# DerryHub/BEVFormer_tensorrt

Measured on AMD Instinct MI355X. Metric: frames/sec BEVFormer-base bs=1 fp16 end-to-end on MI355X (re-hosted model, random weights, synthetic 6-camera frames), higher is better.
Workload: dtype f16

## Files before the change

### bevformer_tensorrt_amd/csrc/capi.hip

```cpp
#include <string.h>

#include "common.h"

extern "C" const char *bevops_version(void) { return "bevops-hip 0.1 (gfx950)"; }

extern "C" const char *bevops_status_string(int status) {
  switch (status) {
    case BEVOPS_SUCCESS: return "success";
    case BEVOPS_FAILURE: return "failure (kernel launch error)";
    case BEVOPS_BAD_PARAM: return "bad parameter";
    case BEVOPS_NOT_SUPPORTED: return "dtype/shape combination not supported";
    case BEVOPS_NOT_INITIALIZED: return "not initialized";
    default: return "unknown status";
  }
}

namespace {
struct Entry {
  const char *name;
  void *fn;
};
const Entry kTable[] = {
    {"bevops_msda_forward", (void *)&bevops_msda_forward},
    {"bevops_msda_forward_ws", (void *)&bevops_msda_forward_ws},
// ... 55 lines not shown
    {"bevops_upsample_bilinear_concat_nhwc", (void *)&bevops_upsample_bilinear_concat_nhwc},
    {"bevops_tsa_split", (void *)&bevops_tsa_split},
    {"bevops_queue_mean2", (void *)&bevops_queue_mean2},
    {"bevops_tsgemm_f16", (void *)&bevops_tsgemm_f16},
    {"bevops_tsgemm_s8", (void *)&bevops_tsgemm_s8},
    {"bevops_tsgemm_s8_ln", (void *)&bevops_tsgemm_s8_ln},
    {"bevops_tsgemm_tile_rows", (void *)&bevops_tsgemm_tile_rows},
    {"bevops_tsgemm_f16_ln", (void *)&bevops_tsgemm_f16_ln},
    {"bevops_tsgemm_f16_grouped", (void *)&bevops_tsgemm_f16_grouped},
    {"bevops_mha_selfattn_f16", (void *)&bevops_mha_selfattn_f16},
    {"bevops_mha_selfattn_max_queries", (void *)&bevops_mha_selfattn_max_queries},
    {"bevops_value_proj_packed_size", (void *)&bevops_value_proj_packed_size},
    {"bevops_value_proj_packed", (void *)&bevops_value_proj_packed},
    {"bevops_value_pack_planes", (void *)&bevops_value_pack_planes},
    {"bevops_sca_prepacked_workspace_size", (void *)&bevops_sca_prepacked_workspace_size},
    {"bevops_sca_forward_prepacked", (void *)&bevops_sca_forward_prepacked},
    {"bevops_sca_plan_size", (void *)&bevops_sca_plan_size},
    {"bevops_sca_plan_build", (void *)&bevops_sca_plan_build},
    {"bevops_sca_forward_planned", (void *)&bevops_sca_forward_planned},
    {"bevops_point_sampling", (void *)&bevops_point_sampling},
    {"bevops_feat_embed_nhwc", (void *)&bevops_feat_embed_nhwc},
    {"bevops_linear_bias_act", (void *)&bevops_linear_bias_act},
    {"bevops_linear_tune", (void *)&bevops_linear_tune},
    {"bevops_quantize_rows", (void *)&bevops_quantize_rows},
    {"bevops_dequantize_rows", (void *)&bevops_dequantize_rows},
    {"bevops_linear_int8", (void *)&bevops_linear_int8},
    {"bevops_linear_int8_fused", (void *)&bevops_linear_int8_fused},
    {"bevops_tile_gemm_f16", (void *)&bevops_tile_gemm_f16},
    {"bevops_tile_gemm_f16_dst", (void *)&bevops_tile_gemm_f16_dst},
    {"bevops_small_gemm_f16_dst", (void *)&bevops_small_gemm_f16_dst},
    {"bevops_small_gemm_f16", (void *)&bevops_small_gemm_f16},
    {"bevops_conv_tile_f16", (void *)&bevops_conv_tile_f16},
    {"bevops_conv3x3_c64_f16", (void *)&bevops_conv3x3_c64_f16},
    {"bevops_refine_reference_points", (void *)&bevops_refine_reference_points},
    {"bevops_decode_boxes", (void *)&bevops_decode_boxes},
    {"bevops_conv_tile_int8_fused", (void *)&bevops_conv_tile_int8_fused},
    {"bevops_linear_int8_chain", (void *)&bevops_linear_int8_chain},
    {"bevops_conv_tile_int8", (void *)&bevops_conv_tile_int8},
    {"bevops_bias_relu_maxpool_nhwc_int8", (void *)&bevops_bias_relu_maxpool_nhwc_int8},
    {"bevops_mdconv_int8_nhwc_workspace_size", (void *)&bevops_mdconv_int8_nhwc_workspace_size},
    {"bevops_mdconv_forward_int8_nhwc", (void *)&bevops_mdconv_forward_int8_nhwc},
    {"bevops_image_normalize_pad", (void *)&bevops_image_normalize_pad},
    {"bevops_image_normalize_resize_pad", (void *)&bevops_image_normalize_resize_pad},
    {"bevops_image_resize_plan_size", (void *)&bevops_image_resize_plan_size},
    {"bevops_image_resize_plan_build", (void *)&bevops_image_resize_plan_build},
    {"bevops_image_resize_crop_normalize", (void *)&bevops_image_resize_crop_normalize},
    {"bevops_msda_packed_size", (void *)&bevops_msda_packed_size},
    {"bevops_msda_pack_value", (void *)&bevops_msda_pack_value},
    {"bevops_msda_forward_prepacked", (void *)&bevops_msda_forward_prepacked},
    {"bevops_linear_workspace_size", (void *)&bevops_linear_workspace_size},
    {"bevops_msda_workspace_size_shapes", (void *)&bevops_msda_workspace_size_shapes},
    {"bevops_sca_workspace_size", (void *)&bevops_sca_workspace_size},
    {"bevops_mdconv_forward_packed", (void *)&bevops_mdconv_forward_packed},
    {"bevops_mdconv_pack_weight", (void *)&bevops_mdconv_pack_weight},
    {"bevops_mdconv_packed_weight_size", (void *)&bevops_mdconv_packed_weight_size},
    {"bevops_conv3x3_c32_pack_weight", (void *)&bevops_conv3x3_c32_pack_weight},
    {"bevops_conv3x3_c32_packed_weight_size", (void *)&bevops_conv3x3_c32_packed_weight_size},
    {"bevops_layer_norm", (void *)&bevops_layer_norm},
    {"bevops_calib_state_size", (void *)&bevops_calib_state_size},
    {"bevops_calib_collect", (void *)&bevops_calib_collect},
    {"bevops_calib_threshold_workspace_size", (void *)&bevops_calib_threshold_workspace_size},
    {"bevops_calib_threshold", (void *)&bevops_calib_threshold},
};
}

extern "C" void *bevops_query(const char *name) {
// ... 6 lines not shown
```

### bevformer_tensorrt_amd/functions/__init__.py

```python
from .multi_scale_deformable_attn import (
    multi_scale_deformable_attn,
    multi_scale_deformable_attn2,
    multi_scale_deformable_attn_int8,
    multi_scale_deformable_attn_local,
    msda_pack_value,
    multi_scale_deformable_attn_prepacked,
)
from .rotate import rotate, rotate2, rotate_int8, rotate_hwc
from .grid_sampler import grid_sampler, grid_sampler2, grid_sampler_int8
from .bev_pool_v2 import bev_pool_v2, bev_pool_v2_2, bev_pool_v2_int8
from .modulated_deformable_conv2d import (modulated_deformable_conv2d, modulated_deformable_conv2d2,
                                          modulated_deformable_conv2d_int8, modulated_deformable_conv2d_nhwc,
                                          bias_act_nhwc_, bias_relu_maxpool_nhwc, conv_offset_nhwc, upsample_add_nhwc_,
                                          feat_embed_nhwc)
from .spatial_cross_attention import (spatial_cross_attention_sample, spatial_cross_attention_projected,
                                      spatial_cross_attention_plan)
from .linear import (linear_bias_act, layer_norm, quantize_rows, dequantize_rows, linear_int8, tsgemm, tsgemm_ln, tsgemm_grouped, tile_gemm, tile_gemm_dst, small_gemm, small_gemm_dst,
                     dense_auto, tsa_split, queue_mean2)
from .int8_chain import linear_int8_chain, linear_int8_ln
from .conv import conv_nhwc, conv3x3_nhwc, conv3x3_auto, conv3x3_c64, conv_int8_nhwc, stem_conv_pool
from .image import (image_normalize_pad, padded_size, bevdet_test_augmentation, bevdet_post_transform, image_resize_plan,
                    image_resize_crop_normalize, BEVFORMER_IMAGE_PIPELINES, scaled_size, scale_lidar2img,
                    image_normalize_resize_pad)
from .point_sampling import point_sampling
from .attention import self_attention_qkv
from .refine import refine_reference_points, decode_boxes
from .multi_head_attn import qkv, qkv2
from .inverse import inverse
from .decode import nms_free_decode, centerpoint_decode
from .nms import bev_nms, nms_bev, circle_nms, bev_iou
from .decode2d import centernet_decode, yolox_decode, box_nms
from .lss_prepare import lss_voxel_prepare, lss_lidar_coor, bev_pool_v2_indirect
from .calibrate import calib_state_size, calib_collect, calib_threshold
from .bev_half import lss_depth_split, upsample_bilinear_concat_nhwc
from ..utils.register import TRT_FUNCTIONS

TRT_FUNCTIONS.register_module(module=multi_scale_deformable_attn)
TRT_FUNCTIONS.register_module(module=multi_scale_deformable_attn2)
TRT_FUNCTIONS.register_module(module=multi_scale_deformable_attn_int8)
for _f in (rotate, rotate2, rotate_int8, grid_sampler, grid_sampler2, grid_sampler_int8,
           bev_pool_v2, bev_pool_v2_2, bev_pool_v2_int8, modulated_deformable_conv2d,
           modulated_deformable_conv2d2, modulated_deformable_conv2d_int8,
           spatial_cross_attention_sample, inverse, qkv, qkv2):
    TRT_FUNCTIONS.register_module(module=_f)

__all__ = [
    "multi_scale_deformable_attn",
    "multi_scale_deformable_attn2",
    "multi_scale_deformable_attn_int8",
    "rotate", "rotate2", "rotate_int8",
    "grid_sampler", "grid_sampler2", "grid_sampler_int8",
    "bev_pool_v2", "bev_pool_v2_2", "bev_pool_v2_int8",
    "modulated_deformable_conv2d", "modulated_deformable_conv2d2", "modulated_deformable_conv2d_int8",
    "inverse", "qkv", "qkv2",
    "nms_free_decode", "centerpoint_decode",
    "bev_nms", "nms_bev", "circle_nms", "bev_iou",
    "centernet_decode", "yolox_decode", "box_nms",
    "lss_voxel_prepare", "lss_lidar_coor", "bev_pool_v2_indirect",
    "calib_state_size", "calib_collect", "calib_threshold",
    "bevdet_test_augmentation", "bevdet_post_transform", "image_resize_plan", "image_resize_crop_normalize",
    "BEVFORMER_IMAGE_PIPELINES", "scaled_size", "scale_lidar2img", "image_normalize_resize_pad",
    "spatial_cross_attention_sample", "spatial_cross_attention_projected", "spatial_cross_attention_plan", "modulated_deformable_conv2d_nhwc", "bias_act_nhwc_", "linear_bias_act", "layer_norm", "rotate_hwc", "conv_offset_nhwc", "upsample_add_nhwc_", "feat_embed_nhwc",
    "msda_pack_value", "multi_scale_deformable_attn_prepacked", "multi_scale_deformable_attn_local", "image_normalize_pad", "padded_size", "quantize_rows", "dequantize_rows", "linear_int8", "tsgemm", "tsgemm_ln", "tsgemm_grouped", "tile_gemm", "tile_gemm_dst", "small_gemm_dst", "small_gemm", "dense_auto", "tsa_split", "queue_mean2", "conv_nhwc", "conv3x3_nhwc", "conv3x3_auto", "conv3x3_c64", "conv_int8_nhwc", "bias_relu_maxpool_nhwc", "stem_conv_pool", "point_sampling", "self_attention_qkv", "refine_reference_points", "decode_boxes",
    "linear_int8_chain", "linear_int8_ln",
    "lss_depth_split", "upsample_bilinear_concat_nhwc",
]
```

### bevformer_tensorrt_amd/functions/conv.py

```python
import os

import torch
import torch.nn.functional as F

from ..utils import lib as _lib
from .modulated_deformable_conv2d import bias_act_nhwc_
from .multi_scale_deformable_attn import _TensorCache

_PACKED = _TensorCache()
_CHOICE = {}
CONV_LOG = []
CONV_MISSES = []
HALO = {"enabled": os.environ.get("BEVOPS_CONV_HALO", "1") == "1"}


def pack_taps(weight):
    hit = _PACKED.get(weight)
    if hit is None:
        hit = _PACKED.put(weight, weight.detach().permute(0, 2, 3, 1).contiguous())
    return hit


def conv_nhwc(x, weight, bias=None, relu=False, residual=None, stride=1):
    assert x.is_cuda and x.dtype == torch.float16 and x.dim() == 4 and weight.shape[2] == weight.shape[3]
    assert x.is_contiguous(memory_format=torch.channels_last)
    B, Cin, H, W = x.shape
    Cout, k = weight.shape[0], weight.shape[2]
    if weight.shape[1] != Cin:
        raise ValueError("weight does not match the input channels")
    wt = pack_taps(weight)
    Ho, Wo = (H + 2 * (k // 2) - k) // stride + 1, (W + 2 * (k // 2) - k) // stride + 1
    out = torch.empty((B, Cout, Ho, Wo), dtype=x.dtype, device=x.device, memory_format=torch.channels_last)
    if residual is not None:
        assert residual.shape == out.shape and residual.dtype == x.dtype
        assert residual.is_contiguous(memory_format=torch.channels_last)
    if bias is not None:
        bias = bias.to(torch.float16).contiguous()
    if B == 0:
        return out
    handle = _lib.load_library()
    with torch.cuda.device(x.device):
        st = handle.bevops_conv_tile_f16(x.data_ptr(), wt.data_ptr(), bias.data_ptr() if bias is not None else None,
                                         residual.data_ptr() if residual is not None else None, out.data_ptr(),
                                         B, H, W, Cin, Cout, k, int(stride), int(bool(relu)),
                                         _lib.current_stream_ptr(x.device))
    _lib.check(st, "bevops_conv_tile_f16")
    return out


def conv3x3_c64(x, weight, bias=None, relu=False, residual=None, stride=1):
    assert x.is_cuda and x.dtype == torch.float16 and x.dim() == 4
    assert x.is_contiguous(memory_format=torch.channels_last)
    B, Cin, H, W = x.shape
    Cout = weight.shape[0]
    if residual is not None or stride != 1 or tuple(weight.shape[1:]) != (Cin, 3, 3):
        raise _lib.BevopsError("bevops_conv3x3_c64_f16: 3x3 / stride 1 layers without identity rows only", _lib.NOT_SUPPORTED)
    wt = pack_taps(weight)
    out = torch.empty((B, Cout, H, W), dtype=x.dtype, device=x.device, memory_format=torch.channels_last)
    if bias is not None:
        bias = bias.to(torch.float16).contiguous()
    if B == 0:
        return out
    handle = _lib.load_library()
    with torch.cuda.device(x.device):
        st = handle.bevops_conv3x3_c64_f16(x.data_ptr(), wt.data_ptr(), bias.data_ptr() if bias is not None else None,
                                           out.data_ptr(), B, H, W, Cin, Cout, int(bool(relu)),
                                           _lib.current_stream_ptr(x.device))
    _lib.check(st, "bevops_conv3x3_c64_f16")
    return out


def conv_int8_nhwc(x, scale_a, w_q_taps, scale_w, bias=None, relu=False, residual=None, stride=1):
    assert x.is_cuda and x.dtype == torch.float16 and x.dim() == 4 and w_q_taps.dtype == torch.int8
    assert x.is_contiguous(memory_format=torch.channels_last) and w_q_taps.is_contiguous()
    B, Cin, H, W = x.shape
    Cout, k = w_q_taps.shape[0], w_q_taps.shape[1]
    assert w_q_taps.shape == (Cout, k, k, Cin)
    Ho, Wo = (H + 2 * (k // 2) - k) // stride + 1, (W + 2 * (k // 2) - k) // stride + 1
    out = torch.empty((B, Cout, Ho, Wo), dtype=x.dtype, device=x.device, memory_format=torch.channels_last)
    if residual is not None:
        assert residual.shape == out.shape and residual.dtype == x.dtype
        assert residual.is_contiguous(memory_format=torch.channels_last)
    per_channel = torch.is_tensor(scale_w)
    ws = scale_w.float().contiguous() if per_channel else None
    b = bias.float().contiguous() if bias is not None else None
    if B == 0:
        return out
    handle = _lib.load_library()
    with torch.cuda.device(x.device):
        st = handle.bevops_conv_tile_int8_fused(
            x.data_ptr(), float(scale_a), w_q_taps.data_ptr(), ws.data_ptr() if per_channel else None,
            1.0 if per_channel else float(scale_w), b.data_ptr() if b is not None else None,
            residual.data_ptr() if residual is not None else None, out.data_ptr(), B, H, W, Cin, Cout, k, int(stride),
            int(bool(relu)), _lib.current_stream_ptr(x.device))
    _lib.check(st, "bevops_conv_tile_int8_fused")
    return out


def conv3x3_nhwc(x, weight, bias=None, relu=False, residual=None, stride=1):
    assert weight.shape[2:] == (3, 3)
    return conv_nhwc(x, weight, bias, relu, residual, stride)


def _library(x, weight, bias, relu, residual, stride=1):
    y = F.conv2d(x, weight, None, stride, weight.shape[2] // 2)
    if not y.is_contiguous(memory_format=torch.channels_last):
        y = y.contiguous(memory_format=torch.channels_last)
    return bias_act_nhwc_(y, bias, residual, relu)


def conv3x3_auto(x, weight, bias=None, relu=False, residual=None, stride=1):
    B, Cin, H, W = x.shape
    if B == 0 and Cin % 32 == 0:
        return conv_nhwc(x, weight, bias, relu, residual, stride)
    key = (str(x.device), B, H, W, Cin, weight.shape[0], weight.shape[2], stride, bool(relu), residual is not None)
    from .linear import DETERMINISTIC, _problem, _table
    halo_ok = HALO["enabled"] and Cin == 64 and weight.shape[0] == 64 and stride == 1 and residual is None \
        and weight.shape[2] == 3
    name = ("halo" if halo_ok else "tile") if (DETERMINISTIC["enabled"] and Cin % 32 == 0) else _CHOICE.get(key)
    if name is None:
        name = _table()["conv"].get(_problem(key))
        if name == "tile" and halo_ok:
            name = "halo"
        if name in ("tile", "library", "halo") and (name == "library" or Cin % 32 == 0) and (name != "halo" or halo_ok):
            _CHOICE[key] = name
        else:
            name = None
            if _problem(key) not in CONV_MISSES:
                CONV_MISSES.append(_problem(key))
    if name is None:
        if Cin % 32 != 0:
            name = _CHOICE[key] = "library"
        elif torch.cuda.is_current_stream_capturing() or os.environ.get("BEVOPS_DENSE_TUNE", "1") == "0":
            name = "library"
        else:
            from .linear import graph_time_us
            times = {}
            for cand, fn in (("tile", conv_nhwc), ("library", _library)) + ((("halo", conv3x3_c64),) if halo_ok else ()):
                for _ in range(2):
                    fn(x, weight, bias, relu, residual, stride)
                torch.cuda.synchronize()
                times[cand] = round(graph_time_us(lambda: fn(x, weight, bias, relu, residual, stride), 4, 3), 1)
            CONV_LOG.append((key, times))
            name = _CHOICE[key] = min(times, key=times.get)
    return {"tile": conv_nhwc, "halo": conv3x3_c64, "library": _library}[name](x, weight, bias, relu, residual, stride)


_STEM_PACKED = _TensorCache()
STEM_FUSED = {"enabled": os.environ.get("BEVOPS_STEM_FUSED", "1") != "0"}


def stem_conv_pool(x, weight, bias=None, scale_out=None):
    assert x.is_cuda and x.dtype == torch.float16 and x.dim() == 4 and x.is_contiguous()
    n, c, h, w = x.shape
    if tuple(weight.shape) != (64, 3, 7, 7) or c != 3 or w % 2:
        raise ValueError("stem_conv_pool: a 7x7 convolution from 3 to 64 channels on images of even width")
    handle = _lib.load_library()
    bstamp = None if bias is None else _TensorCache._stamp(bias)
    hit = _STEM_PACKED.get(weight)
    if hit is None or hit[0] != bstamp:
        wt = weight.detach().to(torch.float16).contiguous()
        bs = None if bias is None else bias.detach().to(torch.float16).contiguous()
        packed = torch.empty(handle.bevops_stem_packed_size(), dtype=torch.uint8, device=x.device)
        with torch.cuda.device(x.device):
            st = handle.bevops_stem_pack(_lib.F16, wt.data_ptr(), bs.data_ptr() if bs is not None else None,
                                         packed.data_ptr(), _lib.current_stream_ptr(x.device))
        _lib.check(st, "bevops_stem_pack")
        hit = _STEM_PACKED.put(weight, (bstamp, packed))
    hc, wc = (h - 1) // 2 + 1, (w - 1) // 2 + 1
    hp, wp = (hc - 1) // 2 + 1, (wc - 1) // 2 + 1
    out = torch.empty((n, 64, hp, wp), dtype=torch.float16 if scale_out is None else torch.int8, device=x.device,
                      memory_format=torch.channels_last)
    if n == 0:
        return out
    with torch.cuda.device(x.device):
        st = handle.bevops_stem_conv_pool(_lib.F16, _lib.F16 if scale_out is None else _lib.I8, x.data_ptr(),
                                          hit[1].data_ptr(), out.data_ptr(), n, h, w,
                                          0.0 if scale_out is None else float(scale_out),
# ... 5 lines not shown
```

### bevformer_tensorrt_amd/functions/linear.py

```python
import ctypes

import torch

from ..utils import lib as _lib
from ..utils import workspace as _ws

def _workspace(device, nbytes, stream):
    return _ws.lend("linear", nbytes, device, stream)


_TUNED = set()


def _tune_once(handle, key, args, x2, out_shape):
    import os
    _TUNED.add(key)
    if os.environ.get("BEVOPS_LINEAR_TUNE", "1") == "0":
        return
    scratch = torch.empty(out_shape, dtype=x2.dtype, device=x2.device)
    a = list(args)
    a[5] = scratch.data_ptr()
    handle.bevops_linear_tune(*a)


# ... 262 lines not shown
class _PerThreadFlag:

    def __init__(self):
        import threading
        self._tls = threading.local()

    def __getitem__(self, key):
        assert key == "enabled"
        return getattr(self._tls, "enabled", False)

    def __setitem__(self, key, value):
        assert key == "enabled"
        self._tls.enabled = bool(value)


DETERMINISTIC = _PerThreadFlag()
OWN_KERNELS = _PerThreadFlag()


_TABLE = {"loaded": False, "dense": {}, "conv": {}, "measured_dense": {}}


def _table():
    import json
    import os
    if not _TABLE["loaded"]:
        _TABLE["loaded"] = True
        path = os.path.join(os.path.dirname(os.path.dirname(os.path.abspath(__file__))), "dispatch_gfx950.json")
        if os.path.exists(path) and os.environ.get("BEVOPS_DENSE_TUNE", "") not in ("0", "1"):
            try:
                t = json.load(open(path))
                _TABLE["dense"], _TABLE["conv"] = t.get("dense", {}), t.get("conv", {})
                _TABLE["measured_dense"] = t.get("measured_us", {}).get("dense", {})
            except (OSError, ValueError):
                pass
    return _TABLE


def _problem(key):
    return ",".join(str(int(v)) if isinstance(v, bool) else str(v) for v in key[1:])


def _small_pays(M, N, K):
    return K % 64 == 0 and K <= 1024 and M * N <= 1024 * 512


def _dense_deterministic(N, K, M=1 << 30):
    if _small_pays(M, N, K):
        return "small"
    return "tsgemm" if (N % 256 == 0 and K % 64 == 0 and K >= 256) else "tile"


def _dense_own(key, N, K, M):
    times = _table().get("measured_dense", {}).get(_problem(key), {})
    own = {k: v for k, v in times.items() if k in ("tile", "tsgemm", "small") and k in _DENSE}
    return min(own, key=own.get) if own else _dense_deterministic(N, K, M)


def own_kernel_choice(device, M, N, K, relu, has_bias, has_res):
    return _dense_own((str(device), M, N, K, bool(relu), bool(has_bias), bool(has_res)), N, K, M)


def _dense_default(N, K, has_res):
    if N == 256 and K % 64 == 0 and K >= 256:
        return "tsgemm"
    return "blaslt"
# ... 104 lines not shown
```

### bevformer_tensorrt_amd/utils/lib.py

```python
import ctypes
import os

_PKG = os.path.dirname(os.path.dirname(os.path.abspath(__file__)))
_LIB = None

c_int, c_float, c_void_p, c_size_t = ctypes.c_int, ctypes.c_float, ctypes.c_void_p, ctypes.c_size_t

SIGNATURES = {
    "bevops_version": (ctypes.c_char_p, []),
    "bevops_status_string": (ctypes.c_char_p, [c_int]),
    "bevops_query": (c_void_p, [ctypes.c_char_p]),
    "bevops_msda_set_variant": (c_int, [c_int]),
    "bevops_msda_forward": (c_int, [c_int, c_void_p, c_void_p, c_void_p, c_void_p, c_int,
                                    c_void_p, c_void_p, c_void_p] + [c_int] * 8 +
                            [c_float] * 4 + [c_void_p]),
    "bevops_msda_workspace_size": (c_size_t, [c_int] * 8),
    "bevops_msda_workspace_size_shapes": (c_size_t, [c_int, c_void_p] + [c_int] * 7),
    "bevops_msda_forward_ws": (c_int, [c_int, c_void_p, c_void_p, c_void_p, c_void_p, c_int,
                                       c_void_p, c_void_p, c_void_p] + [c_int] * 8 +
                               [c_float] * 4 + [c_int, c_void_p, c_size_t, c_void_p]),
    "bevops_msda_packed_size": (c_size_t, [c_int, c_void_p] + [c_int] * 7),
    "bevops_msda_pack_value": (c_int, [c_int, c_int, c_void_p, c_void_p, c_void_p, c_size_t] + [c_int] * 7 + [c_void_p]),
    "bevops_msda_forward_prepacked": (c_int, [c_int, c_void_p, c_size_t, c_void_p, c_void_p, c_int, c_void_p, c_void_p,
                                              c_void_p] + [c_int] * 8 + [c_float] * 4 + [c_int, c_void_p]),
# ... 57 lines not shown
    "bevops_conv3x3_c32_packed_weight_size": (c_size_t, [c_int, c_int]),
    "bevops_conv3x3_c32_pack_weight": (c_int, [c_int, c_void_p, c_void_p, c_int, c_int, c_void_p]),
    "bevops_conv3x3_c32_forward_nhwc": (c_int, [c_int, c_void_p, c_void_p, c_void_p, c_void_p, c_int, c_int, c_int,
                                                c_int, c_void_p]),
    "bevops_rotate_set_variant": (c_int, [c_int]),
    "bevops_rotate_forward_hwc": (c_int, [c_int, c_void_p, c_void_p, c_void_p, c_int, c_void_p,
                                          c_int, c_int, c_int, c_int, c_void_p]),
    "bevops_layer_norm": (c_int, [c_int, c_void_p, c_void_p, c_void_p, c_void_p, c_size_t, c_int, c_float, c_void_p]),
    "bevops_linear_workspace_size": (c_size_t, []),
    "bevops_linear_bias_act": (c_int, [c_int] + [c_void_p] * 5 + [ctypes.c_longlong, c_int, c_int, c_int,
                                                                  c_void_p, c_size_t, c_void_p]),
    "bevops_image_normalize_pad": (c_int, [c_int, c_void_p, c_int, c_void_p] + [c_int] * 5 +
                                   [ctypes.POINTER(ctypes.c_double), ctypes.POINTER(ctypes.c_double), c_int, c_int, c_void_p]),
    "bevops_image_normalize_resize_pad": (c_int, [c_int, c_void_p, c_int, c_void_p] + [c_int] * 7 +
                                          [ctypes.POINTER(ctypes.c_double), ctypes.POINTER(ctypes.c_double), c_int, c_int,
                                           c_void_p]),
    "bevops_image_resize_plan_size": (c_size_t, [c_int] * 8),
    "bevops_image_resize_plan_build": (c_int, [c_int] * 8 + [c_void_p, c_size_t]),
    "bevops_image_resize_crop_normalize": (c_int, [c_void_p, c_void_p, c_size_t, c_int, c_void_p, c_void_p] + [c_int] * 10 +
                                           [ctypes.POINTER(ctypes.c_double), ctypes.POINTER(ctypes.c_double), c_int, c_int,
                                            c_int, c_void_p]),
    "bevops_quantize_rows": (c_int, [c_int, c_void_p, c_void_p, c_size_t, c_float, c_void_p]),
    "bevops_dequantize_rows": (c_int, [c_int, c_void_p, c_void_p, c_size_t, c_float, c_void_p]),
    "bevops_linear_int8": (c_int, [c_void_p, c_float, c_void_p, c_void_p, c_float, c_void_p, c_void_p, c_int, c_void_p,
                                   c_float, ctypes.c_longlong, c_int, c_int, c_int, c_void_p]),
    "bevops_linear_int8_fused": (c_int, [c_void_p, c_float, c_void_p, c_void_p, c_float, c_void_p, c_void_p, c_int, c_void_p,
                                         c_float, ctypes.c_longlong, c_int, c_int, c_int, c_void_p]),
    "bevops_small_gemm_f16": (c_int, [c_void_p] * 5 + [ctypes.c_longlong, c_int, c_int, c_int, c_void_p]),
    "bevops_tile_gemm_f16": (c_int, [c_void_p] * 5 + [ctypes.c_longlong, c_int, c_int, c_int, c_void_p]),
    "bevops_tile_gemm_f16_dst": (c_int, [c_void_p] * 4 + [c_int, ctypes.c_longlong, c_int, c_int, c_int, c_void_p]),
    "bevops_small_gemm_f16_dst": (c_int, [c_void_p] * 4 + [c_int, ctypes.c_longlong, c_int, c_int, c_int, c_void_p]),
    "bevops_conv_tile_f16": (c_int, [c_void_p] * 5 + [c_int] * 8 + [c_void_p]),
    "bevops_conv3x3_c64_f16": (c_int, [c_void_p] * 4 + [c_int] * 6 + [c_void_p]),
    "bevops_refine_reference_points": (c_int, [c_int] + [c_void_p] * 4 + [c_int] * 2 + [c_void_p] * 3),
    "bevops_decode_boxes": (c_int, [c_int] + [c_void_p] * 3 + [c_int] + [c_float] * 6 + [c_void_p] * 3),
    "bevops_bias_relu_maxpool_nhwc": (c_int, [c_int, c_void_p, c_void_p, c_void_p, c_int, c_int, c_int, c_int, c_void_p]),
    "bevops_stem_packed_size": (c_size_t, []),
    "bevops_stem_pack": (c_int, [c_int, c_void_p, c_void_p, c_void_p, c_void_p]),
    "bevops_stem_conv_pool": (c_int, [c_int, c_int, c_void_p, c_void_p, c_void_p, c_int, c_int, c_int, c_float, c_void_p]),
    "bevops_stem_set_variant": (c_int, [c_int]),
    "bevops_conv_tile_int8_fused": (c_int, [c_void_p, c_float, c_void_p, c_void_p, c_float, c_void_p, c_void_p, c_void_p]
                                    + [c_int] * 8 + [c_void_p]),
    "bevops_linear_int8_chain": (c_int, [c_void_p, c_int, c_float, c_void_p, c_void_p, c_float, c_void_p, c_void_p, c_int,
                                         c_float, c_int, c_void_p, c_float, ctypes.c_longlong, c_int, c_int, c_int, c_void_p]),
    "bevops_conv_tile_int8": (c_int, [c_void_p, c_float, c_void_p, c_void_p, c_float, c_void_p, c_void_p, c_int, c_void_p,
                                      c_float] + [c_int] * 8 + [c_void_p]),
    "bevops_bias_relu_maxpool_nhwc_int8": (c_int, [c_int, c_void_p, c_void_p, c_void_p, c_float, c_int, c_int, c_int, c_int,
                                                   c_void_p]),
    "bevops_mdconv_int8_nhwc_workspace_size": (c_size_t, []),
    "bevops_mdconv_forward_int8_nhwc": (c_int, [c_void_p, c_float, c_void_p, c_int, c_float, c_float, c_void_p, c_float,
                                                c_void_p, c_void_p, c_float, c_int, c_int, c_void_p, c_size_t] + [c_int] * 15 +
                                        [c_void_p]),
    "bevops_linear_tune": (c_int, [c_int] + [c_void_p] * 5 + [ctypes.c_longlong, c_int, c_int, c_int,
                                                              c_void_p, c_size_t, c_void_p]),
    "bevops_mdconv_packed_weight_size": (c_size_t, [c_int] * 5),
    "bevops_mdconv_pack_weight": (c_int, [c_int, c_void_p, c_void_p] + [c_int] * 4 + [c_void_p]),
    "bevops_grid_sampler_3d_forward": (c_int, [c_int, c_void_p, c_void_p, c_void_p] + [c_int] * 11 +
                                       [c_void_p]),
    "bevops_qkv_workspace_size": (c_size_t, [c_int] * 5),
    "bevops_qkv_forward": (c_int, [c_int, c_void_p, c_void_p, c_void_p, c_void_p] + [c_int] * 4 + [c_float] * 4 +
                           [c_void_p, c_size_t, c_void_p]),
    "bevops_inverse_forward": (c_int, [c_int, c_void_p, c_void_p, c_int, c_int, c_void_p]),
    "bevops_nms_free_decode": (c_int, [c_int] + [c_void_p] * 6 + [c_int] * 4 + [c_void_p, c_float, c_int, c_void_p]),
    "bevops_centerpoint_decode_workspace_size": (c_size_t, [c_int] * 5),
    "bevops_centerpoint_decode": (c_int, [c_int] + [c_void_p] * 11 + [c_int] * 5 + [c_float] * 5 +
                                  [c_void_p, c_float, c_int, c_int, c_void_p, c_size_t, c_void_p]),
# ... 75 lines not shown
```

### include/bevops.h

```cpp
#ifndef BEVOPS_H_
#define BEVOPS_H_

#include <stddef.h>
#include <stdint.h>

#ifdef __cplusplus
extern "C" {
#endif

typedef enum {
  BEVOPS_SUCCESS = 0,
  BEVOPS_FAILURE = 1,
  BEVOPS_BAD_PARAM = 2,
  BEVOPS_NOT_SUPPORTED = 3,
  BEVOPS_NOT_INITIALIZED = 4
} bevops_status_t;

typedef enum { BEVOPS_F32 = 0, BEVOPS_F16 = 1, BEVOPS_I8 = 2, BEVOPS_U8 = 3  } bevops_dtype_t;

typedef enum { BEVOPS_BILINEAR = 0, BEVOPS_NEAREST = 1, BEVOPS_BICUBIC = 2 } bevops_interp_t;
typedef enum { BEVOPS_PAD_ZEROS = 0, BEVOPS_PAD_BORDER = 1, BEVOPS_PAD_REFLECTION = 2 } bevops_pad_t;

const char *bevops_version(void);
const char *bevops_status_string(int status);
// ... 129 lines not shown
                     void *stream);
int bevops_queue_mean2(int dtype, const void *x, void *out, size_t count, void *stream);
int bevops_rotate_forward_hwc(int dtype, const void *img, const void *angle, const void *center,
                              int angle_dtype, void *output, int channels, int height, int width,
                              int interpolation, void *stream);
int bevops_layer_norm(int dtype, const void *x, const void *gamma, const void *beta, void *out,
                      size_t rows, int channels, float eps, void *stream);
int bevops_quantize_rows(int dtype, const void *x, void *q, size_t count, float scale, void *stream);
int bevops_dequantize_rows(int dtype, const void *q, void *out, size_t count, float scale, void *stream);
int bevops_linear_int8(const void *a_q, float scale_a, const void *w_q, const float *w_scales,
                       float scale_w, const float *bias, const void *residual, int out_dtype,
                       void *out, float scale_out, long long M, int N, int K, int relu, void *stream);
int bevops_linear_int8_fused(const void *x_f16, float scale_a, const void *w_q, const float *w_scales,
                             float scale_w, const float *bias, const void *residual, int out_dtype,
                             void *out, float scale_out, long long M, int N, int K, int relu, void *stream);
int bevops_tile_gemm_f16(const void *x, const void *weight, const void *bias, const void *residual,
                         void *out, long long M, int N, int K, int relu, void *stream);
typedef struct bevops_gemm_dst {
  int col_begin, col_end;
  void *out;
  long long out_pitch;
  const void *res;
  long long res_pitch;
} bevops_gemm_dst;
int bevops_tile_gemm_f16_dst(const void *x, const void *weight, const void *bias, const bevops_gemm_dst *dst, int num_dst,
                             long long M, int N, int K, int relu, void *stream);
int bevops_small_gemm_f16_dst(const void *x, const void *weight, const void *bias, const bevops_gemm_dst *dst, int num_dst,
                              long long M, int N, int K, int relu, void *stream);
int bevops_conv_tile_f16(const void *x, const void *weight_taps, const void *bias, const void *residual,
                         void *out, int B, int H, int W, int Cin, int Cout, int ksize, int stride, int relu,
                         void *stream);
int bevops_conv3x3_c64_f16(const void *x, const void *weight_taps, const void *bias, void *out, int B, int H, int W,
                           int Cin, int Cout, int relu, void *stream);
int bevops_refine_reference_points(int dtype, const void *tmp, const void *reference_points, void *new_reference_points,
                                   void *reference_xy, int num_query, int tmp_stride, const void *log_table,
                                   const void *sigmoid_table, void *stream);
int bevops_decode_boxes(int dtype, const void *regs, const void *refs, void *out, int count, float scale_x, float offset_x,
                        float scale_y, float offset_y, float scale_z, float offset_z, const void *log_table,
                        const void *sigmoid_table, void *stream);
int bevops_conv_tile_int8_fused(const void *x_f16, float scale_a, const void *w_q_taps, const float *w_scales,
                                float scale_w, const float *bias, const void *residual, void *out, int B, int H,
                                int W, int Cin, int Cout, int ksize, int stride, int relu, void *stream);
int bevops_linear_int8_chain(const void *a, int a_dtype, float scale_a, const void *w_q, const float *w_scales,
                             float scale_w, const float *bias, const void *residual, int res_dtype, float scale_res,
                             int out_dtype, void *out, float scale_out, long long M, int N, int K, int relu,
                             void *stream);
int bevops_conv_tile_int8(const void *x_q, float scale_a, const void *w_q_taps, const float *w_scales, float scale_w,
                          const float *bias, const void *residual, int out_dtype, void *out, float scale_out, int B,
                          int H, int W, int Cin, int Cout, int ksize, int stride, int relu, void *stream);
int bevops_bias_relu_maxpool_nhwc_int8(int dtype, const void *x, const void *bias, void *out_q, float scale_out,
                                       int n, int h, int w, int channels, void *stream);
size_t bevops_mdconv_int8_nhwc_workspace_size(void);
int bevops_mdconv_forward_int8_nhwc(const void *input_nhwc, float scale_in, const void *offset_mask_nhwc,
                                    int offset_mask_channels, float scale_offset, float scale_mask,
                                    const void *packed_weight, float scale_weight, const float *bias,
                                    void *output_nhwc, float scale_out, int relu, int exact, void *workspace,
                                    size_t workspace_bytes, int B, int Cin, int H, int W, int Cout, int Kh, int Kw,
                                    int stride_h, int stride_w, int pad_h, int pad_w, int dil_h, int dil_w,
                                    int groups, int deform_groups, void *stream);
int bevops_image_normalize_pad(int in_dtype, const void *images, int out_dtype, void *output, int N,
                               int H0, int W0, int Hp, int Wp, const double *mean_host,
                               const double *std_host, int to_rgb, int channels_last, void *stream);
size_t bevops_image_resize_plan_size(int H0, int W0, int resize_w, int resize_h, int crop_x0, int crop_y0,
                                     int crop_x1, int crop_y1);
int bevops_image_resize_plan_build(int H0, int W0, int resize_w, int resize_h, int crop_x0, int crop_y0, int crop_x1,
                                   int crop_y1, void *plan_host, size_t plan_bytes);
// ... 149 lines not shown
```

Measured before the change: 101.8.

## Add halo-tiled MFMA 3x3 conv kernel for 128/256-channel layers

Adds a new implicit-GEMM 3x3 conv kernel for 128/256 input and output channels. It loads a halo-padded input tile into LDS once and streams swizzled weight slices through a multi-buffered direct-to-LDS pipeline feeding 32x32x16 MFMAs. The epilogue fuses bias, residual and ReLU, then stages results through LDS for coalesced NHWC stores. Dispatch picks this kernel for large enough convs in deterministic mode, or in place of the tiled kernel after autotuning. The risk is that tile and pipeline choices are heuristic, and LDS use is large enough to limit occupancy.

Result: no change. 102.6 (median of 6 runs) (+0.8%).

```diff
diff --git a/bevformer_tensorrt_amd/csrc/capi.hip b/bevformer_tensorrt_amd/csrc/capi.hip
--- a/bevformer_tensorrt_amd/csrc/capi.hip
+++ b/bevformer_tensorrt_amd/csrc/capi.hip
@@ -111,6 +111,7 @@
     {"bevops_small_gemm_f16", (void *)&bevops_small_gemm_f16},
     {"bevops_conv_tile_f16", (void *)&bevops_conv_tile_f16},
     {"bevops_conv3x3_c64_f16", (void *)&bevops_conv3x3_c64_f16},
+    {"bevops_conv3x3_wide_f16", (void *)&bevops_conv3x3_wide_f16},
     {"bevops_refine_reference_points", (void *)&bevops_refine_reference_points},
     {"bevops_decode_boxes", (void *)&bevops_decode_boxes},
     {"bevops_conv_tile_int8_fused", (void *)&bevops_conv_tile_int8_fused},
diff --git a/bevformer_tensorrt_amd/csrc/conv_wide.hip b/bevformer_tensorrt_amd/csrc/conv_wide.hip
--- /dev/null
+++ b/bevformer_tensorrt_amd/csrc/conv_wide.hip
@@ -0,0 +1,300 @@
+#include <algorithm>
+
+#include "common.h"
+
+namespace bevops {
+namespace {
+
+typedef _Float16 f16x8_t __attribute__((ext_vector_type(8)));
+typedef float f32x16_t __attribute__((ext_vector_type(16)));
+typedef __attribute__((address_space(3))) void lds_void;
+
+constexpr int kWTW = 16;
+constexpr int kWLdsMax = 160 * 1024;
+constexpr unsigned kWOob = 0xFFFFFF00u;
+
+template <int CIN, int COUT, int MJ, int KS, int NB>
+struct Wide {
+  static constexpr int kTH = 4 * MJ;
+  static constexpr int kWaves = COUT / 64 * 2, kThreads = kWaves * 64;
+  static constexpr int kPix = CIN * 2 + 16;
+  static constexpr int kRow = ((kWTW + 2) * kPix + 255) / 256 * 256;
+  static constexpr int kXBytes = (kTH + 2) * kRow;
+  static constexpr int kWRow = KS * 2;
+  static constexpr int kCPR = kWRow / 16;
+  static constexpr int kWBuf = COUT * kWRow;
+  static constexpr int kPcW = kWBuf / 1024 / kWaves;
+  static constexpr int kSPix = COUT * 2 + 16;
+  static constexpr int kYBytes = kTH * kWTW * kSPix;
+  static constexpr int kLds = NB * kWBuf + kXBytes > kYBytes ? NB * kWBuf + kXBytes : kYBytes;
+  static constexpr int kStepsTap = CIN / KS, kSteps = 9 * kStepsTap;
+  static constexpr int kCPP = CIN / 8;
+  static constexpr int kChunks = (kTH + 2) * (kWTW + 2) * kCPP;
+  static constexpr int kRounds = (kChunks + kThreads - 1) / kThreads;
+  static constexpr int kOutRounds = kTH * kWTW * (COUT / 8) / kThreads;
+  static constexpr bool kOk = kSteps % NB == 0 && NB * kWBuf <= 64 * 1024 && kLds <= kWLdsMax;
+  static_assert(kPcW * kWaves * 1024 == kWBuf, "");
+};
+
+template <int CPR>
+__device__ __forceinline__ unsigned wide_swz(unsigned row) {
+  return CPR == 8 ? ((row ^ (row >> 3)) & 7u) : ((row >> 2) & 3u);
+}
+
+struct WideArgs {
+  const __half *x, *w, *bias, *res;
+  __half *out;
+  int H, W, relu, tiles_x, tiles_img;
+  unsigned x_bytes;
+};
+
+template <int CIN, int COUT, int MJ, int KS, int NB>
+__global__ __launch_bounds__((Wide<CIN, COUT, MJ, KS, NB>::kThreads)) void conv3x3_wide_kernel(WideArgs p) {
+  using G = Wide<CIN, COUT, MJ, KS, NB>;
+  constexpr int D = NB - 1;
+  extern __shared__ __attribute__((aligned(16))) char smem[];
+  char *Xs = smem + NB * G::kWBuf;
+  const int tid = threadIdx.x, lane = tid & 63, hi = lane >> 5, l31 = lane & 31;
+  const int wave = __builtin_amdgcn_readfirstlane(tid >> 6), cn = wave >> 1, pm = wave & 1;
+  const int H = p.H, W = p.W;
+  const int t = (int)xcd_remap(blockIdx.x, gridDim.x);
+  const int b = t / p.tiles_img, rem = t - b * p.tiles_img;
+  const int ty0 = (rem / p.tiles_x) * G::kTH, tx0 = (rem % p.tiles_x) * kWTW;
+  const __amdgpu_buffer_rsrc_t rs_x = __builtin_amdgcn_make_buffer_rsrc(const_cast<__half *>(p.x), 0, p.x_bytes, 0x00020000);
+  const __amdgpu_buffer_rsrc_t rs_w =
+      __builtin_amdgcn_make_buffer_rsrc(const_cast<__half *>(p.w), 0, (unsigned)(COUT * 9 * CIN * 2), 0x00020000);
+
+  const int first = wave * G::kPcW;
+  unsigned w_off[G::kPcW];
+#pragma unroll
+  for (int j = 0; j < G::kPcW; ++j) {
+    const unsigned pos = (unsigned)((first + j) * 64 + lane), row = pos / G::kCPR;
+    const unsigned c = (pos % G::kCPR) ^ wide_swz<G::kCPR>(row);
+    w_off[j] = row * (unsigned)(9 * CIN * 2) + c * 16u;
+  }
+  auto weights = [&](int step, int buf) __attribute__((always_inline)) {
+#pragma unroll
+    for (int j = 0; j < G::kPcW; ++j)
+      __builtin_amdgcn_raw_ptr_buffer_load_lds(rs_w, (lds_void *)(smem + buf * G::kWBuf + (first + j) * 1024), 16,
+                                               (int)w_off[j], step * (KS * 2), 0, 0);
+  };
+#pragma unroll
+  for (int d = 0; d < D; ++d) weights(d, d);
+
+  {
+    uint4 pre[G::kRounds];
+    int dst[G::kRounds];
+#pragma unroll
+    for (int r = 0; r < G::kRounds; ++r) {
+      const int q = tid + G::kThreads * r, pix = q / G::kCPP, piece = q % G::kCPP;
+      const int hy = pix / (kWTW + 2), hx = pix - hy * (kWTW + 2);
+      const int y = ty0 + hy - 1, xx = tx0 + hx - 1;
+      const bool in = q < G::kChunks && y >= 0 && y < H && xx >= 0 && xx < W;
+      const unsigned off = in ? (unsigned)(((((size_t)b * H + y) * W + xx) * CIN + piece * 8) * 2) : kWOob;
+      pre[r] = __builtin_bit_cast(uint4, __builtin_amdgcn_raw_buffer_load_b128(rs_x, (int)off, 0, 0));
+      dst[r] = q < G::kChunks ? hy * G::kRow + hx * G::kPix + piece * 16 : -1;
+    }
+#pragma unroll
+    for (int r = 0; r < G::kRounds; ++r)
+      if (dst[r] >= 0) *reinterpret_cast<uint4 *>(Xs + dst[r]) = pre[r];
+  }
+
+  const char *wa[2];
+  unsigned ws[2];
+  const char *xb[MJ];
+#pragma unroll
+  for (int i = 0; i < 2; ++i) {
+    const unsigned row = (unsigned)(64 * cn + 32 * i + l31);
+    wa[i] = smem + row * G::kWRow;
+    ws[i] = wide_swz<G::kCPR>(row);
+  }
+#pragma unroll
+  for (int j = 0; j < MJ; ++j)
+    xb[j] = Xs + ((G::kTH / 2) * pm + 2 * j + (l31 >> 4)) * G::kRow + (l31 & 15) * G::kPix + 16 * hi;
+  f32x16_t acc[2][MJ];
+#pragma unroll
+  for (int i = 0; i < 2; ++i)
+#pragma unroll
+    for (int j = 0; j < MJ; ++j)
+#pragma unroll
+      for (int r = 0; r < 16; ++r) acc[i][j][r] = 0.f;
+
+  asm volatile("s_waitcnt vmcnt(0) lgkmcnt(0)" ::: "memory");
+  __builtin_amdgcn_s_barrier();
+
+  for (int s0 = 0; s0 < G::kSteps; s0 += NB) {
+#pragma unroll
+    for (int u = 0; u < NB; ++u) {
+      constexpr int kSub = KS / 16;
+      const int step = s0 + u, tap = step / G::kStepsTap, cs = step % G::kStepsTap;
+      const int xoff = (tap / 3) * G::kRow + (tap % 3) * G::kPix + cs * (KS * 2);
+      weights(step + D, (u + D) % NB);
+      f16x8_t fa[kSub][2], fb[kSub][MJ];
+#pragma unroll
+      for (int kk = 0; kk < kSub; ++kk) {
+#pragma unroll
+        for (int i = 0; i < 2; ++i)
+          fa[kk][i] = *reinterpret_cast<const f16x8_t *>(wa[i] + u * G::kWBuf + ((((unsigned)(2 * kk + hi)) ^ ws[i]) << 4));
+#pragma unroll
+        for (int j = 0; j < MJ; ++j) fb[kk][j] = *reinterpret_cast<const f16x8_t *>(xb[j] + xoff + kk * 32);
+      }
+#pragma unroll
+      for (int kk = 0; kk < kSub; ++kk)
+#pragma unroll
+        for (int i = 0; i < 2; ++i)
+#pragma unroll
+          for (int j = 0; j < MJ; ++j)
+            acc[i][j] = __builtin_amdgcn_mfma_f32_32x32x16_f16(fa[kk][i], fb[kk][j], acc[i][j], 0, 0, 0);
+      asm volatile("s_waitcnt vmcnt(%0) lgkmcnt(0)" ::"n"((D - 1) * G::kPcW) : "memory");
+      __builtin_amdgcn_s_barrier();
+    }
+  }
+  asm volatile("s_waitcnt vmcnt(0)" ::: "memory");
+  __builtin_amdgcn_s_barrier();
+
+#pragma unroll
+  for (int j = 0; j < MJ; ++j) {
+    const int prow = (G::kTH / 2) * pm + 2 * j + (l31 >> 4), pcol = l31 & 15;
+    const int y = ty0 + prow, xx = tx0 + pcol;
+    const bool in = y < H && xx < W;
+    const size_t opix = in ? (((size_t)b * H + y) * W + xx) * COUT : 0;
+    char *srow = smem + (prow * kWTW + pcol) * G::kSPix;
+#pragma unroll
+    for (int i = 0; i < 2; ++i)
+#pragma unroll
+      for (int g = 0; g < 4; ++g) {
+        const int ch = 64 * cn + 32 * i + 8 * g + 4 * hi;
+        const uint2 braw = p.bias ? *reinterpret_cast<const uint2 *>(p.bias + ch) : make_uint2(0u, 0u);
+        float v[4];
+        v[0] = acc[i][j][4 * g] + h2f_lo(braw.x);
+        v[1] = acc[i][j][4 * g + 1] + h2f_hi(braw.x);
+        v[2] = acc[i][j][4 * g + 2] + h2f_lo(braw.y);
+        v[3] = acc[i][j][4 * g + 3] + h2f_hi(braw.y);
+        if (p.res && in) {
+          const uint2 q = *reinterpret_cast<const uint2 *>(p.res + opix + ch);
+          v[0] += h2f_lo(q.x); v[1] += h2f_hi(q.x); v[2] += h2f_lo(q.y); v[3] += h2f_hi(q.y);
+        }
+        if (p.relu) {
+#pragma unroll
+          for (int e = 0; e < 4; ++e) v[e] = fmaxf(v[e], 0.f);
+        }
+        *reinterpret_cast<uint2 *>(srow + ch * 2) = make_uint2(pack_h2(v[0], v[1]), pack_h2(v[2], v[3]));
+      }
+  }
+  __syncthreads();
+#pragma unroll
+  for (int r = 0; r < G::kOutRounds; ++r) {
+    const int q = tid + G::kThreads * r, px = q / (COUT / 8), c = q % (COUT / 8);
+    const int y = ty0 + (px >> 4), xx = tx0 + (px & 15);
+    if (y < H && xx < W)
+      *reinterpret_cast<uint4 *>(p.out + (((size_t)b * H + y) * W + xx) * COUT + c * 8) =
+          *reinterpret_cast<const uint4 *>(smem + px * G::kSPix + c * 16);
+  }
+}
+
+int wide_cu_count() {
+  int dev = 0, cus = 256;
+  if (hipGetDevice(&dev) == hipSuccess) {
+    hipDeviceProp_t p;
+    static int cached[16] = {0};
+    if (cached[dev & 15] == 0 && hipGetDeviceProperties(&p, dev) == hipSuccess) cached[dev & 15] = p.multiProcessorCount;
+    if (cached[dev & 15] > 0) cus = cached[dev & 15];
+  }
+  return cus;
+}
+
+thread_local int g_wide_variant = 0;
+
+constexpr int kWidePipes = 4;
+constexpr int kWidePipe[kWidePipes + 1][2] = {{0, 0}, {32, 3}, {32, 4}, {64, 2}, {64, 3}};
+
+struct WidePlan {
+  int rows = 8, pipe = 1;
+  int tiles_x = 0, tiles_y = 0;
+  long long tiles = 0;
+};
+
+constexpr int wide_lds(int cin, int cout, int rows, int pipe) {
+  const int row = ((kWTW + 2) * (cin * 2 + 16) + 255) / 256 * 256;
+  const int loop = kWidePipe[pipe][1] * cout * kWidePipe[pipe][0] * 2 + (rows + 2) * row, stage = rows * kWTW * (cout * 2 + 16);
+  return loop > stage ? loop : stage;
+}
+constexpr bool wide_ok(int cin, int cout, int rows, int pipe) {
+  return (9 * cin / kWidePipe[pipe][0]) % kWidePipe[pipe][1] == 0 && kWidePipe[pipe][1] * cout * kWidePipe[pipe][0] * 2 <= 64 * 1024 &&
+         wide_lds(cin, cout, rows, pipe) <= kWLdsMax;
+}
+
+bool wide_plan(WidePlan &pl, int B, int H, int W, int cin, int cout) {
+  const int v = g_wide_variant;
+  const int want_rows = (v & 3) == 1 ? 8 : (v & 3) == 2 ? 4 : 0;
+  const int want_pipe = (v >> 2) & 7;
+  auto tiles_of = [&](int rows) { return (long long)B * ((H + rows - 1) / rows) * ((W + kWTW - 1) / kWTW); };
+  pl.rows = want_rows ? want_rows : (tiles_of(8) >= (cin == 128 ? 1ll : 2ll) * wide_cu_count() ? 8 : 4);
+  pl.pipe = cin == 128 ? 1 : 2;
+  if (want_pipe >= 1 && want_pipe <= kWidePipes && wide_ok(cin, cout, pl.rows, want_pipe)) pl.pipe = want_pipe;
+  pl.tiles_x = (W + kWTW - 1) / kWTW;
+  pl.tiles_y = (H + pl.rows - 1) / pl.rows;
+  pl.tiles = tiles_of(pl.rows);
+  return pl.tiles <= (1ll << 30);
+}
+
+template <int CIN, int COUT, int MJ, int KS, int NB>
+int wide_launch(const WideArgs &a, const WidePlan &pl, hipStream_t st) {
+  using G = Wide<CIN, COUT, MJ, KS, NB>;
+  if constexpr (G::kOk) {
+    static_assert(wide_ok(CIN, COUT, G::kTH, KS == 32 ? NB - 2 : NB + 1) && wide_lds(CIN, COUT, G::kTH, KS == 32 ? NB - 2 : NB + 1) == G::kLds, "");
+    if (!ensure_dynamic_lds<conv3x3_wide_kernel<CIN, COUT, MJ, KS, NB>>(G::kLds)) return BEVOPS_FAILURE;
+    hipLaunchKernelGGL((conv3x3_wide_kernel<CIN, COUT, MJ, KS, NB>), dim3((unsigned)pl.tiles), dim3(G::kThreads), G::kLds, st, a);
+    return launch_status();
+  } else {
+    return BEVOPS_FAILURE;
+  }
+}
+
+template <int CIN, int COUT, int MJ>
+int wide_launch_pipe(const WideArgs &a, const WidePlan &pl, hipStream_t st) {
+  switch (pl.pipe) {
+    case 1: return wide_launch<CIN, COUT, MJ, 32, 3>(a, pl, st);
+    case 2: return wide_launch<CIN, COUT, MJ, 32, 4>(a, pl, st);
+    case 3: return wide_launch<CIN, COUT, MJ, 64, 2>(a, pl, st);
+    default: return wide_launch<CIN, COUT, MJ, 64, 3>(a, pl, st);
+  }
+}
+
+template <int CIN, int COUT>
+int wide_launch_shape(const WideArgs &a, const WidePlan &pl, hipStream_t st) {
+  return pl.rows == 8 ? wide_launch_pipe<CIN, COUT, 2>(a, pl, st) : wide_launch_pipe<CIN, COUT, 1>(a, pl, st);
+}
+
+}
+}
+
+using namespace bevops;
+
+extern "C" int bevops_conv3x3_wide_f16(const void *x, const void *weight_taps, const void *bias, const void *residual,
+                                       void *out, int B, int H, int W, int Cin, int Cout, int ksize, int stride, int relu,
+                                       void *stream) {
+  if (!x || !weight_taps || !out || B <= 0 || H <= 0 || W <= 0 || Cin <= 0 || Cout <= 0 || stride <= 0) return BEVOPS_BAD_PARAM;
+  if (ksize != 3 || stride != 1 || (Cin != 128 && Cin != 256) || (Cout != 128 && Cout != 256)) return BEVOPS_NOT_SUPPORTED;
+  if (!aligned16(x) || !aligned16(weight_taps) || !aligned16(out) || (residual && !aligned16(residual)) ||
+      (reinterpret_cast<uintptr_t>(bias) & 7u))
+    return BEVOPS_NOT_SUPPORTED;
+  if ((long long)B * H * W * std::max(Cin, Cout) * 2 >= (long long)kWOob) return BEVOPS_NOT_SUPPORTED;
+  WidePlan pl;
+  if (!wide_plan(pl, B, H, W, Cin, Cout)) return BEVOPS_NOT_SUPPORTED;
+  WideArgs a;
+  a.x = static_cast<const __half *>(x); a.w = static_cast<const __half *>(weight_taps);
+  a.bias = static_cast<const __half *>(bias); a.res = static_cast<const __half *>(residual);
+  a.out = static_cast<__half *>(out);
+  a.H = H; a.W = W; a.relu = relu; a.tiles_x = pl.tiles_x; a.tiles_img = pl.tiles_x * pl.tiles_y;
+  a.x_bytes = (unsigned)((size_t)B * H * W * Cin * 2);
+  hipStream_t st = static_cast<hipStream_t>(stream);
+  if (Cin == 128) return Cout == 128 ? wide_launch_shape<128, 128>(a, pl, st) : wide_launch_shape<128, 256>(a, pl, st);
+  return Cout == 128 ? wide_launch_shape<256, 128>(a, pl, st) : wide_launch_shape<256, 256>(a, pl, st);
+}
+
+extern "C" int bevops_conv3x3_wide_set_variant(int variant) {
+  const int prev = g_wide_variant;
+  g_wide_variant = variant < 0 ? 0 : variant;
+  return prev;
+}
diff --git a/bevformer_tensorrt_amd/functions/__init__.py b/bevformer_tensorrt_amd/functions/__init__.py
--- a/bevformer_tensorrt_amd/functions/__init__.py
+++ b/bevformer_tensorrt_amd/functions/__init__.py
@@ -18,7 +18,7 @@
 from .linear import (linear_bias_act, layer_norm, quantize_rows, dequantize_rows, linear_int8, tsgemm, tsgemm_ln, tsgemm_grouped, tile_gemm, tile_gemm_dst, small_gemm, small_gemm_dst,
                      dense_auto, tsa_split, queue_mean2)
 from .int8_chain import linear_int8_chain, linear_int8_ln
-from .conv import conv_nhwc, conv3x3_nhwc, conv3x3_auto, conv3x3_c64, conv_int8_nhwc, stem_conv_pool
+from .conv import conv_nhwc, conv3x3_nhwc, conv3x3_auto, conv3x3_c64, conv3x3_wide, conv_int8_nhwc, stem_conv_pool
 from .image import (image_normalize_pad, padded_size, bevdet_test_augmentation, bevdet_post_transform, image_resize_plan,
                     image_resize_crop_normalize, BEVFORMER_IMAGE_PIPELINES, scaled_size, scale_lidar2img,
                     image_normalize_resize_pad)
@@ -61,7 +61,7 @@
     "bevdet_test_augmentation", "bevdet_post_transform", "image_resize_plan", "image_resize_crop_normalize",
     "BEVFORMER_IMAGE_PIPELINES", "scaled_size", "scale_lidar2img", "image_normalize_resize_pad",
     "spatial_cross_attention_sample", "spatial_cross_attention_projected", "spatial_cross_attention_plan", "modulated_deformable_conv2d_nhwc", "bias_act_nhwc_", "linear_bias_act", "layer_norm", "rotate_hwc", "conv_offset_nhwc", "upsample_add_nhwc_", "feat_embed_nhwc",
-    "msda_pack_value", "multi_scale_deformable_attn_prepacked", "multi_scale_deformable_attn_local", "image_normalize_pad", "padded_size", "quantize_rows", "dequantize_rows", "linear_int8", "tsgemm", "tsgemm_ln", "tsgemm_grouped", "tile_gemm", "tile_gemm_dst", "small_gemm_dst", "small_gemm", "dense_auto", "tsa_split", "queue_mean2", "conv_nhwc", "conv3x3_nhwc", "conv3x3_auto", "conv3x3_c64", "conv_int8_nhwc", "bias_relu_maxpool_nhwc", "stem_conv_pool", "point_sampling", "self_attention_qkv", "refine_reference_points", "decode_boxes",
+    "msda_pack_value", "multi_scale_deformable_attn_prepacked", "multi_scale_deformable_attn_local", "image_normalize_pad", "padded_size", "quantize_rows", "dequantize_rows", "linear_int8", "tsgemm", "tsgemm_ln", "tsgemm_grouped", "tile_gemm", "tile_gemm_dst", "small_gemm_dst", "small_gemm", "dense_auto", "tsa_split", "queue_mean2", "conv_nhwc", "conv3x3_nhwc", "conv3x3_auto", "conv3x3_c64", "conv3x3_wide", "conv_int8_nhwc", "bias_relu_maxpool_nhwc", "stem_conv_pool", "point_sampling", "self_attention_qkv", "refine_reference_points", "decode_boxes",
     "linear_int8_chain", "linear_int8_ln",
     "lss_depth_split", "upsample_bilinear_concat_nhwc",
 ]
diff --git a/bevformer_tensorrt_amd/functions/conv.py b/bevformer_tensorrt_amd/functions/conv.py
--- a/bevformer_tensorrt_amd/functions/conv.py
+++ b/bevformer_tensorrt_amd/functions/conv.py
@@ -10,8 +10,11 @@
 _PACKED = _TensorCache()
 _CHOICE = {}
 CONV_LOG = []
+_MEASURED = set()
 CONV_MISSES = []
 HALO = {"enabled": os.environ.get("BEVOPS_CONV_HALO", "1") == "1"}
+WIDE = {"enabled": os.environ.get("BEVOPS_CONV_WIDE", "1") == "1"}
+WIDE_MIN_PIXELS = 4000
 
 
 def pack_taps(weight):
@@ -70,6 +73,37 @@
     return out
 
 
+def wide_domain(Cin, Cout, ksize, stride):
+    return Cin in (128, 256) and Cout in (128, 256) and ksize == 3 and stride == 1
+
+
+def conv3x3_wide(x, weight, bias=None, relu=False, residual=None, stride=1):
+    assert x.is_cuda and x.dtype == torch.float16 and x.dim() == 4 and weight.shape[2] == weight.shape[3]
+    assert x.is_contiguous(memory_format=torch.channels_last)
+    B, Cin, H, W = x.shape
+    Cout, k = weight.shape[0], weight.shape[2]
+    if weight.shape[1] != Cin:
+        raise ValueError("weight does not match the input channels")
+    if not wide_domain(Cin, Cout, k, stride) or B == 0:
+        return conv_nhwc(x, weight, bias, relu, residual, stride)
+    wt = pack_taps(weight)
+    out = torch.empty((B, Cout, H, W), dtype=x.dtype, device=x.device, memory_format=torch.channels_last)
+    if residual is not None:
+        assert residual.shape == out.shape and residual.dtype == x.dtype
+        assert residual.is_contiguous(memory_format=torch.channels_last)
+    b16 = bias.to(torch.float16).contiguous() if bias is not None else None
+    handle = _lib.load_library()
+    with torch.cuda.device(x.device):
+        st = handle.bevops_conv3x3_wide_f16(x.data_ptr(), wt.data_ptr(), b16.data_ptr() if b16 is not None else None,
+                                            residual.data_ptr() if residual is not None else None, out.data_ptr(),
+                                            B, H, W, Cin, Cout, k, int(stride), int(bool(relu)),
+                                            _lib.current_stream_ptr(x.device))
+    if st == _lib.NOT_SUPPORTED:
+        return conv_nhwc(x, weight, bias, relu, residual, stride)
+    _lib.check(st, "bevops_conv3x3_wide_f16")
+    return out
+
+
 def conv_int8_nhwc(x, scale_a, w_q_taps, scale_w, bias=None, relu=False, residual=None, stride=1):
     assert x.is_cuda and x.dtype == torch.float16 and x.dim() == 4 and w_q_taps.dtype == torch.int8
     assert x.is_contiguous(memory_format=torch.channels_last) and w_q_taps.is_contiguous()
@@ -117,12 +151,19 @@
     from .linear import DETERMINISTIC, _problem, _table
     halo_ok = HALO["enabled"] and Cin == 64 and weight.shape[0] == 64 and stride == 1 and residual is None \
         and weight.shape[2] == 3
-    name = ("halo" if halo_ok else "tile") if (DETERMINISTIC["enabled"] and Cin % 32 == 0) else _CHOICE.get(key)
+    wide_ok = WIDE["enabled"] and wide_domain(Cin, weight.shape[0], weight.shape[2], stride)
+    if DETERMINISTIC["enabled"] and Cin % 32 == 0:
+        name = "halo" if halo_ok else ("wide" if wide_ok and B * H * W >= WIDE_MIN_PIXELS else "tile")
+    else:
+        name = _CHOICE.get(key)
     if name is None:
         name = _table()["conv"].get(_problem(key))
         if name == "tile" and halo_ok:
             name = "halo"
-        if name in ("tile", "library", "halo") and (name == "library" or Cin % 32 == 0) and (name != "halo" or halo_ok):
+        if name in ("tile", "library") and wide_domain(Cin, weight.shape[0], weight.shape[2], stride) \
+                and _table().get("conv_wide", {}).get(_problem(key)) == "wide":
+            name = "wide"
+        if name in ("tile", "library", "halo", "wide") and (name == "library" or Cin % 32 == 0) and (name != "halo" or halo_ok):
             _CHOICE[key] = name
         else:
             name = None
@@ -143,7 +184,13 @@
                 times[cand] = round(graph_time_us(lambda: fn(x, weight, bias, relu, residual, stride), 4, 3), 1)
             CONV_LOG.append((key, times))
             name = _CHOICE[key] = min(times, key=times.get)
-    return {"tile": conv_nhwc, "halo": conv3x3_c64, "library": _library}[name](x, weight, bias, relu, residual, stride)
+            _MEASURED.add(key)
+    if name == "tile" and key in _MEASURED and wide_ok and B * H * W >= WIDE_MIN_PIXELS:
+        name = "wide"
+    if name == "wide" and not wide_ok:
+        name = "tile"
+    return {"tile": conv_nhwc, "halo": conv3x3_c64, "wide": conv3x3_wide, "library": _library}[name](
+        x, weight, bias, relu, residual, stride)
 
 
 _STEM_PACKED = _TensorCache()
diff --git a/bevformer_tensorrt_amd/functions/linear.py b/bevformer_tensorrt_amd/functions/linear.py
--- a/bevformer_tensorrt_amd/functions/linear.py
+++ b/bevformer_tensorrt_amd/functions/linear.py
@@ -318,6 +318,7 @@
                 t = json.load(open(path))
                 _TABLE["dense"], _TABLE["conv"] = t.get("dense", {}), t.get("conv", {})
                 _TABLE["measured_dense"] = t.get("measured_us", {}).get("dense", {})
+                _TABLE["conv_wide"] = t.get("conv_wide", {})
             except (OSError, ValueError):
                 pass
     return _TABLE
diff --git a/bevformer_tensorrt_amd/utils/lib.py b/bevformer_tensorrt_amd/utils/lib.py
--- a/bevformer_tensorrt_amd/utils/lib.py
+++ b/bevformer_tensorrt_amd/utils/lib.py
@@ -113,6 +113,8 @@
     "bevops_small_gemm_f16_dst": (c_int, [c_void_p] * 4 + [c_int, ctypes.c_longlong, c_int, c_int, c_int, c_void_p]),
     "bevops_conv_tile_f16": (c_int, [c_void_p] * 5 + [c_int] * 8 + [c_void_p]),
     "bevops_conv3x3_c64_f16": (c_int, [c_void_p] * 4 + [c_int] * 6 + [c_void_p]),
+    "bevops_conv3x3_wide_f16": (c_int, [c_void_p] * 5 + [c_int] * 8 + [c_void_p]),
+    "bevops_conv3x3_wide_set_variant": (c_int, [c_int]),
     "bevops_refine_reference_points": (c_int, [c_int] + [c_void_p] * 4 + [c_int] * 2 + [c_void_p] * 3),
     "bevops_decode_boxes": (c_int, [c_int] + [c_void_p] * 3 + [c_int] + [c_float] * 6 + [c_void_p] * 3),
     "bevops_bias_relu_maxpool_nhwc": (c_int, [c_int, c_void_p, c_void_p, c_void_p, c_int, c_int, c_int, c_int, c_void_p]),
diff --git a/include/bevops.h b/include/bevops.h
--- a/include/bevops.h
+++ b/include/bevops.h
@@ -185,6 +185,9 @@
                          void *stream);
 int bevops_conv3x3_c64_f16(const void *x, const void *weight_taps, const void *bias, void *out, int B, int H, int W,
                            int Cin, int Cout, int relu, void *stream);
+int bevops_conv3x3_wide_f16(const void *x, const void *weight_taps, const void *bias, const void *residual, void *out,
+                            int B, int H, int W, int Cin, int Cout, int ksize, int stride, int relu, void *stream);
+int bevops_conv3x3_wide_set_variant(int variant);
 int bevops_refine_reference_points(int dtype, const void *tmp, const void *reference_points, void *new_reference_points,
                                    void *reference_xy, int num_query, int tmp_stride, const void *log_table,
                                    const void *sigmoid_table, void *stream);
```
